# Enigmatisms/AdaPT

Measured on AMD Instinct MI355X. Metric: Msamples/s (W*H*spp/s), unidirectional MIS path tracing, higher is better.
Workload: dtype f32

## Files before the change

### adapt_amd/_lib.py

```python
from __future__ import annotations

import ctypes as C
import os

_HERE = os.path.dirname(os.path.abspath(__file__))
LIB_PATHS = {"fast": os.environ.get("ADAPT_MI_LIB") or os.path.join(_HERE, "libadapt_mi.so"),
             "exact": os.environ.get("ADAPT_MI_LIB_EXACT") or os.path.join(_HERE, "libadapt_mi_exact.so")}
_variant = "exact" if os.environ.get("APT_EXACT", "0") not in ("", "0") else "fast"
LIB_PATH = LIB_PATHS[_variant]

f32p = C.POINTER(C.c_float)
i32p = C.POINTER(C.c_int32)
u32p = C.POINTER(C.c_uint32)
u8p = C.POINTER(C.c_uint8)
f64p = C.POINTER(C.c_double)
APT_N_KERNELS = 5
KERNEL_NAMES = ("generate", "extend", "shade", "shadow", "finalize")


class AptError(RuntimeError):
    pass


class SceneDesc(C.Structure):
# ... 58 lines not shown
    "apt_read_pixels": (C.c_int, [C.c_void_p, f32p]),
    "apt_get_accum": (C.c_int, [C.c_void_p, f32p, i32p]),
    "apt_set_accum": (C.c_int, [C.c_void_p, f32p, C.c_int32]),
    "apt_reset": (C.c_int, [C.c_void_p]),
    "apt_read_transient": (C.c_int, [C.c_void_p, f32p]),
    "apt_set_transient": (C.c_int, [C.c_void_p, f32p]),
    "apt_read_sample_counts": (C.c_int, [C.c_void_p, i32p, u8p]),
    "apt_read_moments": (C.c_int, [C.c_void_p, f64p]),
    "apt_set_adaptive_state": (C.c_int, [C.c_void_p, i32p, f64p, u8p]),
    "apt_get_stats": (C.c_int, [C.c_void_p, C.POINTER(Stats)]),
    "apt_device_ptr": (C.c_int, [C.c_void_p, C.POINTER(C.c_void_p), i32p]),
    "apt_stream": (C.c_int, [C.c_void_p, C.POINTER(C.c_void_p)]),
    "apt_intersect": (C.c_int, [C.c_void_p, C.c_int32, f32p, f32p, i32p, f32p, f32p]),
    "apt_occluded": (C.c_int, [C.c_void_p, C.c_int32, f32p, f32p, f32p, i32p]),
    "apt_rng_stream": (C.c_int, [C.c_int32, C.c_uint32, C.c_uint32, C.c_uint32, C.c_int32, u32p]),
    "apt_bxdf_probe": (C.c_int, [C.c_int32, C.c_int32, i32p, f32p, f32p, C.c_float, C.c_int32, C.c_uint32, f32p]),
    "apt_medium_probe": (C.c_int, [C.c_int32, C.c_int32, i32p, f32p, C.c_int32, f32p, C.c_uint32, f32p]),
    "apt_volume_probe": (C.c_int, [C.c_int32, C.c_int32, i32p, f32p, f32p, C.c_int32, f32p, C.c_uint32, f32p]),
    "apt_emitter_probe": (C.c_int, [C.c_void_p, C.c_int32, f32p, C.c_uint32, f32p]),
    "apt_texture_probe": (C.c_int, [C.c_void_p, C.c_int32, i32p, f32p, f32p]),
    "apt_transient_bin_probe": (C.c_int, [C.c_int32, C.c_int32, f32p, C.c_float, C.c_float, C.c_int32, i32p]),
    "apt_renderer_info": (C.c_int, [C.c_void_p, i32p, i32p, C.POINTER(C.c_int64), i32p, C.POINTER(C.c_char_p), i32p]),
    "apt_renderer_camera_fused": (C.c_int, [C.c_void_p, i32p]),
    "apt_measure_sclk_mhz": (C.c_int, [C.c_int32, f32p]),
    "apt_last_error": (C.c_char_p, []),
    "apt_version": (C.c_char_p, []),
}

_libs = {}


def use(variant: str) -> str:
    global _variant, LIB_PATH
    if variant not in LIB_PATHS:
        raise ValueError(f"unknown build variant {variant!r}")
    prev, _variant = _variant, variant
    LIB_PATH = LIB_PATHS[variant]
    return prev


def variant() -> str:
    return _variant


def load(variant: str | None = None):
    v = variant or _variant
# ... 28 lines not shown
```

### adapt_amd/csrc/api.hip

```cpp
#include <hip/hip_runtime.h>
#include <chrono>

#include <algorithm>
#include <cmath>
#include <cstdio>
#include <cstdlib>
#include <cstring>
#include <limits>
#include <memory>
#include <string>
#include <vector>

#include "../../include/adapt_mi.h"
#include "bvh_build.hpp"
#include "shade_stage.hpp"
#include "unit_kernels.hpp"
#include "volumetric.hpp"

#define APT_EXPORT extern "C" __attribute__((visibility("default")))

static thread_local std::string g_err;
static int fail(int code, const std::string& msg) { g_err = msg; return code; }
#define HIP_TRY(expr)                                                                              \
    do {                                                                                           \
// ... 130 lines not shown
struct EventPair { hipEvent_t a, b; int kernel; bool own_a; };

struct Lane {
    hipStream_t stream = nullptr;
    DevBuf pool, counters, ovf;
    Queues q{};
    hipEvent_t fin = nullptr;
    LdsPlan plan{};
    Counters* cnt() const { return counters.as<Counters>(); }
};

struct apt_renderer {
    const apt_scene* scene = nullptr;
    apt_render_cfg cfg{};
    Params par{};
    int n_cols = 0, npix = 0, spp_batch = 1;
    int cnt = 0;
    std::vector<Lane> lanes;
    int n_lanes = 1;
    hipStream_t stream() const { return lanes[0].stream; }
    DevBuf accum, scratch, pix_key;
    DevBuf cam_strips;
    int camera_fuse = 0;
    Counters host_counters{};
    int grid_small = 0, grid_trace = 0, nq = APT_MAX_NQ;
    const ShadeVariant* shade = nullptr;
    int trace_mode = 0;
    int trace_nt = BLOCK;
    int trace_items = BLOCK;
    int sorted = 0;
    int volumetric = 0;
    int dyn_fetch = 0;
    bool tile_ok = false;
    extend_fn extend = nullptr, fix = nullptr;
    int ovf_levels = 0;
    int v_ncls = 0;
    int vev_single = 0;
    vev_shade_fn vev_all = nullptr;
    bool vev_live[APT_MAX_CLASSES] = {};
    vev_group_fn vgroup_fn[APT_N_VGROUPS] = {};
    int vgroup_cls[APT_N_VGROUPS][4] = {};
    group_fn group_fn_[APT_N_GROUPS] = {};
    int group_cls[APT_N_GROUPS][APT_GROUP_SLOTS] = {};
    std::string shade_name;
    size_t lds_bytes = 0, lds_bytes_any = 0;
    int grid_shadow = 0;
// ... 554 lines not shown
    r->extend = r->dyn_fetch ? kExtendDyn[r->sorted] : (r->trace_mode == 3 ? kExtendFlatHot[r->sorted] : kExtend[r->trace_mode][r->sorted]);
    r->fix = kFixFlat[r->sorted];
    return APT_OK;
}

static apt::CamFilm cam_film(const apt_render_cfg& c) {
    apt::CamFilm cf;
    memcpy(cf.cam_r, c.cam_r, sizeof(cf.cam_r)); memcpy(cf.cam_t, c.cam_t, sizeof(cf.cam_t));
    cf.inv_focal = c.inv_focal; cf.half_w = c.half_w; cf.half_h = c.half_h;
    cf.width = c.width; cf.height = c.height; cf.n_cols = owned_columns(c); cf.band_width = c.band_width; cf.rank = c.rank; cf.world = c.world_size;
    return cf;
}
static int make_camera_strips(apt_renderer* r) {
    if (r->par.fused != 2) return APT_OK;
    const apt_scene* sc = r->scene;
    const bool cull = !(getenv("APT_CAMERA_CULL") && atoi(getenv("APT_CAMERA_CULL")) == 0);
    std::vector<uint64_t> masks;
    if (apt::camera_strips(sc->h_prims.data(), sc->n_prims, sc->h_flat_recs, sc->h_flat_tab, sc->h_flat_counts, cam_film(r->cfg), cull, masks) != 0)
        return fail(APT_E_INVALID, "apt_renderer_create: camera strip lists: bad record or film");
    hipError_t e = upload(r->cam_strips, masks);
    if (e != hipSuccess) return fail(APT_E_HIP, std::string("upload camera strip lists: ") + hipGetErrorString(e));
    const bool want = !(getenv("APT_CAMERA_FUSE") && atoi(getenv("APT_CAMERA_FUSE")) == 0);
    r->camera_fuse = (want && !r->adaptive && !r->par.do_crop && r->par.max_bounce >= 1 && r->shade->traced_cam != nullptr) ? 1 : 0;
    return APT_OK;
}

APT_EXPORT int apt_camera_strips(const float* prims, int32_t n_prims, const int32_t* obj_info, int32_t n_objects, const apt_render_cfg* cfg, int32_t cull,
                                 uint64_t* masks, int32_t masks_cap, int32_t* n_strips, int32_t* n_pairs) {
    if (!prims || !obj_info || !cfg || n_prims <= 0 || n_objects <= 0 || !n_strips || !n_pairs) return fail(APT_E_INVALID, "apt_camera_strips: bad argument");
    apt_render_cfg c = *cfg;
    if (c.world_size <= 0) { c.world_size = 1; c.rank = 0; }
    if (c.band_width <= 0) c.band_width = c.width;
    if (c.width <= 0 || c.height <= 0 || c.rank < 0 || c.rank >= c.world_size || owned_columns(c) <= 0) return fail(APT_E_INVALID, "apt_camera_strips: bad film or rank");
    std::vector<float> st, tb; int cn[7];
    if (apt::build_flat(prims, n_prims, obj_info, n_objects, nullptr, st, tb, cn) != 0) return fail(APT_E_INVALID, "apt_camera_strips: obj_info range outside the primitive array");
    std::vector<uint64_t> m;
    if (apt::camera_strips(prims, n_prims, st, tb, cn, cam_film(c), cull != 0, m) != 0) return fail(APT_E_INVALID, "apt_camera_strips: bad record or film");
    *n_strips = (int32_t)m.size();
    *n_pairs = (cn[0] + cn[1] + 1) / 2 + (cn[2] + cn[3] + 1) / 2 + (cn[4] + cn[5] + 1) / 2 + (cn[6] + 1) / 2;
    if (masks) { if (masks_cap < (int32_t)m.size()) return fail(APT_E_INVALID, "apt_camera_strips: masks buffer too small"); memcpy(masks, m.data(), m.size() * 8); }
    return APT_OK;
}

static int make_lanes(apt_renderer* r) {
    const apt_scene* sc = r->scene;
    const Params& p = r->par;
// ... 203 lines not shown
    if (c.band_width <= 0) c.band_width = c.width;
    if (c.rank < 0 || c.rank >= c.world_size) return fail(APT_E_INVALID, "apt_renderer_create: rank outside world_size");
    if (c.device != sc->device) return fail(APT_E_INVALID, "apt_renderer_create: renderer and scene must live on the same device");
    if (c.transient_bins < 0) return fail(APT_E_INVALID, "apt_renderer_create: transient_bins must be >= 0 (0 = steady state)");
    if (c.transient_bins > 0) {
        if (c.volumetric) return fail(APT_E_INVALID, "apt_renderer_create: transient rendering is a surface-renderer mode (volumetric = 0)");
        if (c.num_shadow_ray > 4) return fail(APT_E_INVALID, "apt_renderer_create: transient rendering takes at most 4 light samples per vertex (num_shadow_ray <= 4)");
        if (c.world_size > 1) return fail(APT_E_INVALID, "apt_renderer_create: transient rendering runs on one rank (world_size = 1)");
        if (!(c.transient_interval > 0.f) || !std::isfinite(c.transient_interval) || !std::isfinite(c.transient_min_time))
            return fail(APT_E_INVALID, "apt_renderer_create: transient_interval must be positive and finite, transient_min_time finite");
    }
    if (!std::isfinite(c.adaptive_threshold)) return fail(APT_E_INVALID, "apt_renderer_create: adaptive_threshold must be finite (> 0: adaptive sampling, <= 0: off)");
    if (c.adaptive_threshold > 0.f) {
        if (c.transient_bins > 0)
            return fail(APT_E_INVALID, "apt_renderer_create: adaptive sampling and transient rendering do not combine (transient_bins must be 0 when adaptive_threshold > 0)");
        if (c.adaptive_min_spp <= 0 || c.adaptive_step <= 0)
            return fail(APT_E_INVALID, "apt_renderer_create: adaptive sampling needs adaptive_min_spp > 0 and adaptive_step > 0");
    }
    HIP_TRY(hipSetDevice(c.device));
    apt_renderer* r = new apt_renderer();
    struct Owner { apt_renderer* r; ~Owner() { if (r) apt_renderer_destroy(r); } } owner{r};
    r->scene = sc; r->cfg = c;
    r->adaptive = c.adaptive_threshold > 0.f ? 1 : 0;
    if (int rc = plan_film(r)) return rc;
    pick_traversal(r);
    if (int rc = pick_shading(r)) return rc;
    if (int rc = make_camera_strips(r)) return rc;
    if (int rc = make_lanes(r)) return rc;
    if (int rc = make_transient(r)) return rc;
    if (int rc = make_adaptive(r)) return rc;
    if (int rc = plan_lds_and_grids(r)) return rc;
    if (int rc = make_overflow_stacks(r)) return rc;
    for (Lane& ln : r->lanes) HIP_TRY(hipStreamSynchronize(ln.stream));
    owner.r = nullptr;
    *out = r;
    return APT_OK;
}

static int grid_for(size_t n, int cap_blocks, int nq, int nt = BLOCK) {
    size_t b = (n + nt - 1) / nt;
    b = ((b + nq - 1) / nq) * nq;
    if (b < (size_t)nq) b = nq;
    return (int)(b < (size_t)cap_blocks ? b : (size_t)cap_blocks);
}

static void unchain(apt_renderer* r, hipStream_t st) {
// ... 32 lines not shown
        r->kernel_ms[ev.kernel] += ms;
    }
    for (auto& ev : r->pending) { if (ev.own_a) r->free_events.push_back(ev.a); r->free_events.push_back(ev.b); }
    r->pending.clear();
    r->chain.clear();
    if (r->render_pending) {
        float ms = 0.f;
        HIP_TRY(hipEventElapsedTime(&ms, r->ev_r0, r->ev_r1));
        r->render_ms += ms; r->render_pending = false;
    }
    return APT_OK;
}

static int lane_batch(const apt_renderer* r, int32_t n_spp) {
    if (n_spp <= 0) return 1;
    int n_batches = (n_spp + r->spp_batch - 1) / r->spp_batch;
    n_batches = ((n_batches + r->n_lanes - 1) / r->n_lanes) * r->n_lanes;
    return std::max(1, std::min(r->spp_batch, (n_spp + n_batches - 1) / n_batches));
}

static int begin_batch(apt_renderer* r, Lane& ln) {
    unchain(r, ln.stream);
    HIP_TRY(hipMemsetAsync(ln.cnt(), 0, offsetof(Counters, stats), ln.stream));
    return APT_OK;
}
static void launch_extend(apt_renderer* r, Lane& ln, const Params& p, size_t total, int cur) {
    const DevScene& sc = r->scene->dev;
    Counters* cnt = ln.cnt();
    { LaunchTimer t(r, 1, ln.stream); hipLaunchKernelGGL(r->extend, dim3(grid_for(total, r->grid_trace, r->nq, r->trace_items)), dim3(r->trace_nt), r->lds_bytes, ln.stream, sc, p, ln.q, cnt, cur, (const uint32_t*)cnt->n_active[cur], ln.plan); }
    if (r->trace_mode == 3) { LaunchTimer t(r, 1, ln.stream, false); hipLaunchKernelGGL(r->fix, dim3(r->grid_fix), dim3(BLOCK), 0, ln.stream, sc, p, ln.q, cnt, cur, (const uint32_t*)cnt->n_active[cur], ln.plan); }
}
static int finalize_batch(apt_renderer* r, Lane& ln, const Params& p, hipEvent_t& prev_fin) {
    if (prev_fin && r->n_lanes > 1) { unchain(r, ln.stream); HIP_TRY(hipStreamWaitEvent(ln.stream, prev_fin, 0)); }
    {
        LaunchTimer t(r, 4, ln.stream);
        if (r->adaptive) hipLaunchKernelGGL(k_finalize_ad, dim3(grid_for((size_t)r->npix, r->grid_small, 1)), dim3(BLOCK), 0, ln.stream, p, ln.q, r->accum.as<float>(), r->aq);
        else hipLaunchKernelGGL(k_finalize, dim3(grid_for((size_t)r->npix, r->grid_small, 1)), dim3(BLOCK), 0, ln.stream, p, ln.q, r->accum.as<float>());
    }
    HIP_TRY(hipEventRecord(ln.fin, ln.stream));
    prev_fin = ln.fin;
    HIP_TRY(hipGetLastError());
    return APT_OK;
}

static int render_volumetric(apt_renderer* r, int32_t n_spp) {
    const DevScene& sc = r->scene->dev;
// ... 539 lines not shown
    int ndev = 0;
    if (int rc = count_device(&ndev)) return rc;
    if (device < 0 || device >= ndev) return fail(APT_E_INVALID, "apt_measure_sclk_mhz: device ordinal out of range");
    HIP_TRY(hipSetDevice(device));
    hipDeviceProp_t prop;
    HIP_TRY(hipGetDeviceProperties(&prop, device));
    const int grid = std::max(1, prop.multiProcessorCount) * 8, n_waves = grid * (BLOCK / 64);
    DevBuf out, sink;
    HIP_TRY(out.alloc((size_t)n_waves * 16)); HIP_TRY(sink.alloc(16));
    for (int pass = 0; pass < 2; pass++) {
        hipLaunchKernelGGL(k_clock_probe, dim3(grid), dim3(BLOCK), 0, 0, 20000, 1.0f, out.as<unsigned long long>(), sink.as<float>());
        HIP_TRY(hipGetLastError());
        HIP_TRY(hipDeviceSynchronize());
    }
    std::vector<unsigned long long> h((size_t)n_waves * 2);
    HIP_TRY(hipMemcpy(h.data(), out.p, h.size() * 8, hipMemcpyDeviceToHost));
    std::vector<double> r;
    for (int w = 0; w < n_waves; w++) if (h[2 * (size_t)w + 1] > 0) r.push_back(100.0 * (double)h[2 * (size_t)w] / (double)h[2 * (size_t)w + 1]);
    if (r.empty()) return fail(APT_E_STATE, "apt_measure_sclk_mhz: the wall clock did not advance");
    std::nth_element(r.begin(), r.begin() + r.size() / 2, r.end());
    *mhz = (float)r[r.size() / 2];
    return APT_OK;
}
APT_EXPORT int apt_renderer_camera_fused(const apt_renderer* r, int32_t* fused) {
    if (!r || !fused) return fail(APT_E_INVALID, "apt_renderer_camera_fused: null argument");
    *fused = r->camera_fuse;
    return APT_OK;
}
APT_EXPORT int apt_renderer_info(const apt_renderer* r, int32_t* spp_batch, int32_t* n_subqueues, int64_t* queue_bytes, int32_t* lds_bytes, const char** shade_variant, int32_t* trace_mode) {
    if (!r) return fail(APT_E_INVALID, "apt_renderer_info: null handle");
    if (spp_batch) *spp_batch = r->spp_batch;
    if (n_subqueues) *n_subqueues = r->nq;
    if (queue_bytes) *queue_bytes = (int64_t)r->lanes[0].pool.bytes * (int64_t)r->lanes.size();
    if (lds_bytes) *lds_bytes = (int32_t)r->lds_bytes;
    if (shade_variant) *shade_variant = r->shade_name.c_str();
    if (trace_mode) *trace_mode = r->trace_mode;
    return APT_OK;
}
```

### adapt_amd/csrc/shade_stage.hpp

```cpp
#pragma once
#include "stages.hpp"

APT_D float ti_fmod(float a, float b) { float q = floorf(a / b); return a - b * q; }
APT_D f3 mix3(f3 a, f3 b, float t) { return a * (1.0f - t) + b * t; }
APT_D f3 texture_query(const DevScene& sc, int map, int obj, float u, float v) {
    const int* ti_ = sc.tex_i + 15 * obj + 5 * map; const float* tf = sc.tex_f + 6 * obj + 2 * map;
    const float w = (float)ti_[3], h = (float)ti_[4];
    const float scaled_u = ti_fmod((u * tf[0]) * w, w - 1.f), scaled_v = ti_fmod((v * tf[1]) * h, h - 1.f);
    float floor_u = floorf(scaled_u), floor_v = floorf(scaled_v);
    const float ratio_u = scaled_u - floor_u, ratio_v = scaled_v - floor_v;
    floor_u = floor_u + (float)ti_[1]; floor_v = floor_v + (float)ti_[2];
    const int fu = (int)floor_u, fv = (int)floor_v;
    const float* img = sc.atlas[map]; const int W = sc.atlas_w[map];
    const float* r0 = img + ((size_t)fv * W + fu) * 3; const float* r1 = r0 + (size_t)W * 3;
    const f3 q_ff = mk3(r0[0], r0[1], r0[2]), q_cf = mk3(r0[3], r0[4], r0[5]), q_fc = mk3(r1[0], r1[1], r1[2]), q_cc = mk3(r1[3], r1[4], r1[5]);
    return mix3(mix3(q_ff, q_cf, ratio_u), mix3(q_fc, q_cc, ratio_u), ratio_v);
}
APT_D bool get_uv_item(const DevScene& sc, int map, int obj, int prim, float bu, float bv, f3& out) {
    if (sc.atlas[map] == nullptr || !(sc.tex_i[15 * obj + 5 * map] > -255)) return false;
    const float* uv = sc.uvs + 6 * prim;
    const float w0 = 1.f - bu - bv;
    const float gu = (uv[2] * bu + uv[4] * bv) + uv[0] * w0, gv = (uv[3] * bu + uv[5] * bv) + uv[1] * w0;
    out = texture_query(sc, map, obj, gu, gv);
    return true;
// ... 37 lines not shown
        if (lane_id() == 0) old = atomicMax(&cnt->fix_claim[sq * CNT_PAD], epoch);
        old = (uint32_t)__builtin_amdgcn_readlane((int)old, 0);
    }
    if (old >= epoch) {
        while (__hip_atomic_load(&cnt->fix_done[sq * CNT_PAD], __ATOMIC_ACQUIRE, __HIP_MEMORY_SCOPE_AGENT) < epoch) __builtin_amdgcn_s_sleep(16);
        return;
    }
    const uint32_t qbase = (uint32_t)sq * p.subcap, sh_qbase = (uint32_t)sq * q.sh_subcap;
    const bool need_uv = sc.has_vn || sc.tex_i != nullptr;
    for (uint32_t base = 0; base < n_def; base += 64u) {
        const uint32_t li = base + lane_id(); const bool valid = li < n_def;
        const uint32_t lj = valid ? li : n_def - 1u;
        const uint32_t io = (q.tr_stage_top ? qbase + p.subcap - n_def + lj : (uint32_t)ncls * p.cap + qbase + lj) << 4;
        const float4 ra = ldq(q.tr[cur][0], io), rb = ldq(q.tr[cur][1], io), rc = ldq(q.tr[cur][2], io), rd = ldq(q.tr[cur][3], io);
        const f3 o = mk3(ra.x, ra.y, ra.z), d = mk3(rb.x, rb.y, rb.z);
        HitRec r0, r1; r0.t = r1.t = 1e7f; r0.prim = r1.prim = -1; r0.u = r0.v = r1.u = r1.v = 0.f;
        int c0, c1;
        flat_closest2(sc.flat, sc.sweep, sc.prim_class, o, d, o, d, r0, r1, c0, c1);
        if (valid && r0.prim >= 0) {
            const int oc = ncls > 1 ? c0 : 0;
            const uint32_t pos = atomicAdd(&cnt->n_tr[bounce % 3][oc][sq * CNT_PAD], 1u);
            const uint32_t slot = (uint32_t)oc * p.cap + qbase + pos, so = slot << 4;
            stq(q.tr[cur][0], so, make_float4(ra.x, ra.y, ra.z, r0.t));
            stq(q.tr[cur][1], so, make_float4(rb.x, rb.y, rb.z, __uint_as_float((__float_as_uint(rb.w) & ~0xffu) | (uint32_t)r0.prim)));
            stq(q.tr[cur][2], so, rc); stq(q.tr[cur][3], so, rd);
            if (need_uv) { float2 uv_; uv_.x = r0.u; uv_.y = r0.v; stq(q.tr_uv[cur], slot << 3, uv_); }
        } else if (valid && !(rd.x == 0.f && rd.y == 0.f && rd.z == 0.f)) {
            const uint32_t id = __float_as_uint(rc.w), lp_ = id & ((1u << p.pix_bits) - 1u), s_ = id >> p.pix_bits;
            add_radiance(q.L, p.cap, (s_ * (uint32_t)p.npix + lp_) << 2, mk3(rd.x, rd.y, rd.z), true);
        }
    }
    uint32_t t_lit = 0;
    for (uint32_t base = 0; base < n_sh; base += 64u) {
        const uint32_t li = base + lane_id(); const bool valid = li < n_sh;
        const uint32_t io = (sh_qbase + (valid ? li : n_sh - 1u)) << 2;
        const f3 o = ld3q(q.sh_o, q.sh_cap, io), d = ld3q(q.sh_d, q.sh_cap, io), c = ld3q(q.sh_c, q.sh_cap, io);
        const float dist = ldq(q.sh_tmax, io); const uint32_t slot = ldq(q.sh_id, io);
        bool occ, occ_b;
        const float lim = (dist > 0.0f) ? dist - 1e-4f : 1e7f;
        flat_any2(sc.flat, sc.sweep, o, d, o, d, lim, lim, occ, occ_b);
        const bool weird = !(isfinite(c.x) && isfinite(c.y) && isfinite(c.z));
        const bool add = valid && (!occ || weird);
        for (unsigned long long m = __ballot(add); m != 0ull; m &= m - 1ull) {
            if ((int)lane_id() == __ffsll((long long)m) - 1) add_radiance(q.L, p.cap, slot, occ ? c * 0.f : c, true);
        }
        t_lit += (valid && !occ) ? 1u : 0u;
    }
    flush_stat(t_lit, &cnt->stats[sq][ST_LIT]);
    if (lane_id() == 0) __hip_atomic_store(n_sh_p, 0u, __ATOMIC_RELAXED, __HIP_MEMORY_SCOPE_AGENT);
    __threadfence();
    if (lane_id() == 0) __hip_atomic_store(&cnt->fix_done[sq * CNT_PAD], epoch, __ATOMIC_RELEASE, __HIP_MEMORY_SCOPE_AGENT);
}
// ... 153 lines not shown
    uint32_t n, cam_total = 0;
    if constexpr (CAM) {
        cam_total = (uint32_t)(A_->p).npix * (uint32_t)(A_->p).spp_batch;
        const uint32_t n_waves = (cam_total + 63u) / 64u, nq_ = (uint32_t)(A_->p).nq;
        n = n_waves > (uint32_t)sl.q ? ((n_waves - (uint32_t)sl.q + nq_ - 1u) / nq_) * 64u : 0u;
    } else {
        fix_prologue((A_->sc), (A_->p), (A_->q), cnt, cur, sl.q, bounce);
        n = __hip_atomic_load(&cnt->n_tr[bounce % 3][0][sl.q * CNT_PAD], __ATOMIC_RELAXED, __HIP_MEMORY_SCOPE_AGENT);
    }
    uint32_t pf_pm = 0;
    auto prefetch_prim = [&](uint32_t b) { pf_pm = ldq(reinterpret_cast<const uint32_t*>(trB), ((qbase + min(b + threadIdx.x, n - 1u)) << 4) + 12u); };
    if (PFP && n > 0) prefetch_prim(sl.first);
    for (uint32_t base = sl.first; base < n; base += sl.stride) {
        APT_ARGS_PHASE();
        const uint32_t pos = base + threadIdx.x, idx = qbase + pos;
        bool alive = pos < n;
        const uint32_t cu_pm = pf_pm;
        float4 cu_ra = make_float4(0.f, 0.f, 0.f, 0.f), cu_rb = cu_ra;
        if (PFP) { const int rp = max(tr_prim(cu_pm), 0); cu_ra = (A_->sc).prim_shade[2 * rp]; cu_rb = (A_->sc).prim_shade[2 * rp + 1]; prefetch_prim(base + sl.stride); }
        Vertex vx; vertex_reset(vx);
        Rng rng; rng_init(rng, 0u, 0u, 0u, 0u);
        f3 Lc = splat3(0.f);
        bool entry = alive;
        float ray_pdf = 1.f;
        if constexpr (CAM) {
            const uint32_t w = (uint32_t)__builtin_amdgcn_readfirstlane((int)(pos >> 6)) * (uint32_t)(A_->p).nq + (uint32_t)sl.q;
            const uint32_t id_ = w * 64u + lane_id();
            const bool valid = alive && id_ < cam_total;
            f3 dir = mk3(0.f, 0.f, 1.f);
            uint32_t draws = 0;
            uint32_t jitter_tail[2] = {0u, 0u};
            if (valid) {
                const uint32_t lp = id_ % (uint32_t)(A_->p).npix, s = id_ / (uint32_t)(A_->p).npix;
                int i, j; local_to_global((A_->p), lp, i, j);
                for (int pl = 0; pl < (A_->p).l_planes; pl++) stL((A_->q).L, (A_->p).cap, (id_ << 2) | (uint32_t)pl, splat3(0.f));
                dir = camera_ray_dir((A_->p), i, j, s, draws, (WINDOW && APT_DRAW_WINDOW_CARRY) ? jitter_tail : nullptr);
                vx.id = (s << (A_->p).pix_bits) | lp;
            }
            if (draws) atomicAdd(&s_draws[threadIdx.x >> 6], draws);
            const f3 cam_o = mk3((A_->p).cam_t[0], (A_->p).cam_t[1], (A_->p).cam_t[2]);
            float c_t = 0.f; int c_run = -1, c_idx = -1;
            if (__any(valid)) c_idx = flat_closest1<true>((A_->sc).flat, cam_o, dir, 1e7f, c_t, c_run, camera_strip_mask((A_->p), strips, w));
            const bool c_defer = valid && (c_run >= 0 || flat_needs_cull((A_->sc).flat, dir));
            HitRec hr; hr.t = 1e7f; hr.prim = -1; hr.u = hr.v = 0.f;
            int hit_cls = 0;
            if (valid && !c_defer && c_idx >= 0) flat_resolve((A_->sc).flat, c_idx, c_t, cam_o, dir, hr, hit_cls);
            { const uint32_t nv = wave_count(valid); t_samples += nv; t_extend += nv; }
            if (__any(c_defer)) {
                const int ncls = (A_->q).tr_ncls;
                const uint32_t dpos = wave_append(c_defer, &cnt->n_tr[0][ncls][sl.q * CNT_PAD]);
                if (c_defer) {
                    const uint32_t slot = (A_->q).tr_stage_top ? qbase + (A_->p).subcap - 1u - dpos : (uint32_t)ncls * (A_->p).cap + qbase + dpos, so = slot << 4;
                    stq((A_->q).tr[0][0], so, make_float4(cam_o.x, cam_o.y, cam_o.z, hr.t));
                    stq((A_->q).tr[0][1], so, make_float4(dir.x, dir.y, dir.z, __uint_as_float(tr_pack(hr.prim, draws, false))));
                    stq((A_->q).tr[0][2], so, make_float4(1.f, 1.f, 1.f, __uint_as_float(vx.id)));
                    float one = 1.f;
                    if (WINDOW) asm volatile("" : "+v"(one));
                    stq((A_->q).tr[0][3], so, make_float4(0.f, 0.f, 0.f, one));
                    if ((A_->sc).has_vn || (A_->sc).tex_i != nullptr) { float2 uv_; uv_.x = hr.u; uv_.y = hr.v; stq((A_->q).tr_uv[0], slot << 3, uv_); }
                }
            }
            entry = valid && !c_defer;
            alive = entry && hr.prim >= 0;
            if (alive) {
                vx.o = cam_o; vx.d = dir; vx.thr = splat3(1.f);
                f3 rec_kd; float2 uv; uv.x = hr.u; uv.y = hr.v;
                build_hit((A_->sc), hr.prim, hr.t, uv.x, uv.y, vx.o, vx.d, vx.it, vx.hit_light, rec_kd);
                alive = open_vertex<BM, SM, TEX>(A_, vx, rng, hr.prim, rec_kd, tr_meta(tr_pack(hr.prim, draws, false), 0u), ray_pdf, uv, 0, (WINDOW && APT_DRAW_WINDOW_CARRY) ? jitter_tail : nullptr);
            }
        }
        if (!CAM && alive && bounce > 0) { const float4 dd = ldq(trD, idx << 4); Lc = mk3(dd.x, dd.y, dd.z); if (SM & 2) ray_pdf = dd.w; }
        if (!CAM && alive) {
            const float4 a = ldq(trA, idx << 4), b_ = ldq(trB, idx << 4), c = ldq(trC, idx << 4);
            vx.o = mk3(a.x, a.y, a.z); vx.d = mk3(b_.x, b_.y, b_.z); vx.thr = mk3(c.x, c.y, c.z); vx.id = __float_as_uint(c.w);
            const uint32_t pm = PFP ? cu_pm : __float_as_uint(b_.w);
            const int prim = tr_prim(pm);
            if (prim < 0) alive = false;
            else {
                f3 rec_kd; float2 uv; uv.x = uv.y = 0.f;
                if ((A_->sc).has_vn || (TEX && (A_->sc).tex_i != nullptr)) uv = ldq((A_->q).tr_uv[cur], idx << 3);
                if (PFP) build_hit_rec((A_->sc), cu_ra, cu_rb, prim, a.w, uv.x, uv.y, vx.o, vx.d, vx.it, vx.hit_light, rec_kd);
                else build_hit((A_->sc), prim, a.w, uv.x, uv.y, vx.o, vx.d, vx.it, vx.hit_light, rec_kd);
                alive = open_vertex<BM, SM, TEX>(A_, vx, rng, prim, rec_kd, tr_meta(pm, (uint32_t)bounce), ray_pdf, uv, bounce);
            }
        }
        tl.shade += wave_count(alive);
#ifdef APT_NEAR_STATS
        t_near += wave_count(alive && bounce > 0 && vx.it.min_depth < 2e-3f);
#endif
        if (alive) vx.hit_point = vx.d * vx.it.min_depth + vx.o;

        APT_ARGS_PHASE();
        bool break_flag = false;
        DevSrc src_only;
        if ((A_->sc).n_sources == 1) src_only = ld_src_uniform((A_->sc).src);
        const LightSample f = sample_light<BM, SM, false>(A_, vx, rng, geom, src_only, alive, break_flag);
        if (f.poisoned) Lc = splat3(f.mis_w);
        tl.shadow += wave_count(f.sampled); tl.poison += wave_count(f.poisoned);
        int occ_e = 0;
        if ((A_->sc).n_sources != 1) {
            const unsigned long long wm = __ballot(f.want);
            occ_e = -1;
            if (wm != 0ull) {
                const int e0 = __builtin_amdgcn_readlane(f.src, __ffsll((long long)wm) - 1);
                if (!__any(f.want && f.src != e0)) occ_e = e0;
            }
        }
        APT_ARGS_PHASE();
        bool cont = false, is_spec = false;
        f3 new_d = mk3(0.f, 1.f, 0.f);
        float new_pdf = 1.f;
        if (alive) {
            new_d = emit_and_scatter<BM, SM>(A_, vx, rng, new_pdf, is_spec, [&](f3 add) { Lc = Lc + add; });
            cont = (bounce + 1) < (A_->p).max_bounce;
        }
        if (rng.draw != vx.draw0) atomicAdd(&s_draws[threadIdx.x >> 6], rng.draw - vx.draw0);
        APT_ARGS_PHASE();
        float tr_t = 0.f; int tr_hit = -1; float tr_u = 0.f, tr_v = 0.f; int tr_q = -1;
        TrAppend tr_app; tr_app.raw = 0u; tr_app.rank = 0u;
        {
            int tr_idx = -1, tr_run = -1, hit_cls = 0;
            if (__any(cont)) tr_idx = flat_closest1((A_->sc).flat, vx.hit_point, new_d, 1e7f, tr_t, tr_run);
            const bool tr_defer = cont && (tr_run >= 0 || flat_needs_cull((A_->sc).flat, new_d));
            t_extend += wave_count(cont);
            cont = cont && (tr_idx >= 0 || tr_defer);
            if (cont && !tr_defer) { HitRec hr; flat_resolve((A_->sc).flat, tr_idx, tr_t, vx.hit_point, new_d, hr, hit_cls); tr_hit = hr.prim; tr_u = hr.u; tr_v = hr.v; }
            tr_q = !cont ? -1 : (tr_defer ? 1 : 0);
            { const Append a_ = append_issue(tr_q == 0, next_counter); tr_app.raw = a_.raw; tr_app.rank = rank_in(a_.m); }
        }
        APT_ARGS_PHASE();
        {
            const bool defer = f.want && flat_needs_cull((A_->sc).flat, f.dir);
            bool occ = false;
            if (__any(f.want && !defer)) {
                const FlatList ls = (occ_e >= 0) ? flat_occ_list((A_->sc).flat, occ_e) : flat_full_list((A_->sc).flat);
                occ = flat_any1(ls, vx.hit_point, f.dir, (f.dist > 0.0f) ? f.dist - 1e-4f : 1e7f);
            }
            if (__any(defer)) {
                const uint32_t spos = wave_append(defer, &cnt->n_fix_sh[cur][sl.q * CNT_PAD]);
                if (defer && spos < (A_->q).sh_subcap) { const uint32_t so = (sh_qbase + spos) << 2; shadow_store((A_->q), so, vx.hit_point, f.dir, f.dist, f.contrib); stq((A_->q).sh_id, so, vx.l_off); }
            }
            const bool traced = f.want && !defer;
            if (traced) {
                const bool weird = !(isfinite(f.contrib.x) && isfinite(f.contrib.y) && isfinite(f.contrib.z));
                if (!occ || weird) Lc = Lc + (occ ? f.contrib * 0.f : f.contrib);
            }
            t_traced += wave_count(f.want); t_lit += wave_count(traced && !occ);
        }
        uint32_t npos = (uint32_t)__builtin_amdgcn_readlane((int)tr_app.raw, 0) + tr_app.rank;
        if (__any(tr_q == 1)) { const uint32_t dpos = wave_append(tr_q == 1, next_counter + APT_MAX_NQ * CNT_PAD); if (tr_q == 1) npos = dpos; }
        if (cont) {
            const uint32_t slot = (tr_q == 1) ? qbase + (A_->p).subcap - 1u - npos : qbase + npos, so = slot << 4;
            stq((A_->q).tr[nxt][0], so, make_float4(vx.hit_point.x, vx.hit_point.y, vx.hit_point.z, tr_t));
            stq((A_->q).tr[nxt][1], so, make_float4(new_d.x, new_d.y, new_d.z, __uint_as_float(tr_pack(tr_hit, rng.draw, is_spec))));
            stq((A_->q).tr[nxt][2], so, make_float4(vx.thr.x, vx.thr.y, vx.thr.z, __uint_as_float(vx.id)));
            stq((A_->q).tr[nxt][3], so, make_float4(Lc.x, Lc.y, Lc.z, new_pdf));
            if ((A_->sc).has_vn || (A_->sc).tex_i != nullptr) { float2 uv_; uv_.x = tr_u; uv_.y = tr_v; stq((A_->q).tr_uv[nxt], slot << 3, uv_); }
        }
        if (!cont && entry && !(Lc.x == 0.f && Lc.y == 0.f && Lc.z == 0.f)) {
            const uint32_t lp_ = vx.id & ((1u << (A_->p).pix_bits) - 1u), s_ = vx.id >> (A_->p).pix_bits;
            add_radiance((A_->q).L, (A_->p).cap, (s_ * (uint32_t)(A_->p).npix + lp_) << 2, Lc, true);
        }
    }
    flush_uniform(t_traced, &cnt->stats[sl.q][ST_SHADOW_TRACED]); flush_uniform(t_lit, &cnt->stats[sl.q][ST_LIT]);
    flush_uniform(t_extend, &cnt->stats[sl.q][ST_EXTEND]);
    if (CAM) flush_uniform(t_samples, &cnt->stats[sl.q][ST_SAMPLES]);
    tally_flush(tl, s_draws, cnt, sl.q);
#ifdef APT_NEAR_STATS
    flush_uniform(t_near, &cnt->stats[sl.q][14]);
#endif
}
#endif
template <int BM, int SM, int TEX, bool CQ, bool TR = false>
APT_D void shade_staged(args3_ptr A0, Counters* cnt, const ShadeIn& in, int cur, int bounce, TransQ tq = TransQ{}) {
    const ShadeArgs3* A_ = args_fresh(A0);
    const int nxt = cur ^ 1;
    const SubLoop sl = sub_loop((A_->p).nq);
    const uint32_t n = in.counts[sl.q * CNT_PAD];
    const uint32_t qbase = (uint32_t)sl.q * (A_->p).subcap, sh_qbase = (uint32_t)sl.q * (A_->q).sh_subcap;
    uint32_t* next_counter = &cnt->n_active[nxt][sl.q * CNT_PAD];
    uint32_t* shadow_counter = &cnt->n_shadow[sl.q * CNT_PAD];
    const EmitterGeom geom = {(A_->sc).precom, (A_->sc).normals, (A_->sc).obj_info};
    __shared__ uint32_t s_draws[BLOCK / 64];
    if (lane_id() == 0) s_draws[threadIdx.x >> 6] = 0;
// ... 164 lines not shown
```

### adapt_amd/csrc/stages.hpp

```cpp
#pragma once
#include <hip/hip_runtime.h>

#include "rng.hpp"
#include "shading.hpp"
#include "traverse.hpp"
#include "vec.hpp"

struct DevMedium {
    int type;
    float ior;
    f3 u_s, u_a, u_e, par, pdf;
};
struct DevVolume {
    int type, xres, yres, zres;
    f3 albedo, trans, mini, maxi, majorant, pdf;
    f3 inv_r0, inv_r1, inv_r2;
    DevMedium ph;
    const float* grid;
};
struct DevScene {
    DevBvh bvh;
    SweepScene sweep;
    FlatScene flat;
    const float* normals;
// ... 21 lines not shown
    float cam_r[9], cam_t[3];
    float inv_focal, half_w, half_h;
    int W, H, n_cols, npix;
    int band_width, rank, world;
    int do_crop, sx, ex, sy, ey;
    int max_bounce, S;
    float inv_S;
    int use_rr, use_mis, anti_alias, stratified, two_sides, rr_bounce_th;
    float rr_threshold;
    uint32_t seed;
    int cnt_base, spp_batch;
    uint32_t cap;
    uint32_t subcap;
    int nq;
    uint32_t pix_bits;
    const uint32_t* pix_key;
    float inv_ns, inv_ns1;
    int fix_par;
    int volumetric_flat;
    int nee_vm;
    int l_planes;
    int fused;
    float w_min[3], w_max[3];
};

struct Queues {
    float* ray_o[2]; float* ray_d[2];
    float* hit_t; int* hit_prim; float* hit_u; float* hit_v;
    float4* tr[2][4]; float2* tr_uv[2]; int tr_ncls, tr_stage_top;
    uint32_t* fix_ext; uint32_t* fix_sh;
    float* thr[2]; uint32_t* id[2]; uint32_t* meta[2]; float* pdf[2];
    float* sh_o; float* sh_d; float* sh_tmax; float* sh_c; uint32_t* sh_id;
    uint32_t* sh_walk[2];
    float* L;
    uint32_t sh_cap, sh_subcap;
    float4* cq[4];
    int n_classes;
};
#define APT_MAX_CLASSES 8
struct TransQ {
    float* t_path;
    float4* emit;
    float* t_light;
    float4* bins;
    int n_bins;
    float min_time, interval, max_time;
};
// ... 10 lines not shown

#ifndef APT_MAX_NQ
#define APT_MAX_NQ 32
#endif
#define CNT_PAD 32
enum { ST_SAMPLES = 0, ST_EXTEND, ST_SHADE, ST_SHADOW, ST_SHADOW_TRACED, ST_LIT, ST_DRAWS, ST_POISON, ST_TRACK, ST_OVERFLOW, ST_COUNT };
struct Counters {
    uint32_t n_active[2][APT_MAX_NQ * CNT_PAD];
    uint32_t n_shadow[APT_MAX_NQ * CNT_PAD];
    uint32_t n_walk[8][APT_MAX_NQ * CNT_PAD];
    uint32_t n_cls[8][APT_MAX_NQ * CNT_PAD];
    uint32_t n_fix_ext[2][APT_MAX_NQ * CNT_PAD];
    uint32_t n_fix_sh[2][APT_MAX_NQ * CNT_PAD];
    uint32_t n_work[2][APT_MAX_NQ * CNT_PAD];
    uint32_t n_tr[3][8 + 1][APT_MAX_NQ * CNT_PAD];
    uint32_t fix_claim[APT_MAX_NQ * CNT_PAD];
    uint32_t fix_done[APT_MAX_NQ * CNT_PAD];
    unsigned long long stats[APT_MAX_NQ][16];
#ifdef APT_WALK_STATS
    unsigned long long wdbg[2][8];
#endif
};

APT_D uint32_t pack_meta(uint32_t draw, uint32_t bounce, bool spec) { return (draw & 0xffffu) | ((bounce & 0xffu) << 16) | (spec ? (1u << 24) : 0u); }

#define BLOCK 256
#define TR_NO_PRIM 0xffu
APT_D uint32_t tr_pack(int prim, uint32_t draw, bool spec) { return (prim < 0 ? TR_NO_PRIM : (uint32_t)prim) | ((draw & 0xffffu) << 8) | (spec ? (1u << 24) : 0u); }
APT_D int tr_prim(uint32_t pm) { return ((pm & 0xffu) == TR_NO_PRIM) ? -1 : (int)(pm & 0xffu); }
APT_D uint32_t tr_meta(uint32_t pm, uint32_t bounce) { return pack_meta(pm >> 8, bounce, ((pm >> 24) & 1u) != 0u); }
#ifndef APT_EXCLUSIVE_L
#define APT_EXCLUSIVE_L(p) ((p).S == 1 || (p).l_planes == (p).S)
#endif

struct LdsPlan { int stack_depth; uint2* ovf; int ovf_stride; };
extern __shared__ float4 s_dyn[];
typedef __attribute__((address_space(3))) float lds_f;
APT_D TravStack make_stack(const LdsPlan& plan) {
    TravStack ts;
    ts.lds = (lds_u2*)(reinterpret_cast<grp_t*>(s_dyn)) + threadIdx.x;
    ts.stride = BLOCK; ts.k = plan.stack_depth; ts.ovf_stride = plan.ovf_stride;
    ts.ovf = plan.ovf ? (glb_u2*)(reinterpret_cast<grp_t*>(plan.ovf) + (blockIdx.x * blockDim.x + threadIdx.x)) : (glb_u2*)nullptr;
    ts.lut = (lds_u8*)nullptr;
    return ts;
}
APT_D TravStack make_walk_stack(const LdsPlan& plan) {
    TravStack ts = make_stack(plan);
    ts.lut = (lds_u8*)(reinterpret_cast<float*>(s_dyn) + (size_t)plan.stack_depth * BLOCK * 2 + 6 * BLOCK);
    fill_permute_lut(ts.lut);
    __syncthreads();
    return ts;
}

// ... 840 lines not shown
```

### adapt_amd/renderer.py

```python
from __future__ import annotations

import ctypes as C
import time
from typing import List, Optional

import numpy as np

from . import _lib
from .scene_pack import FlatScene, RenderConfig, make_config, pack_scene
from .tiles import TilePlan

__all__ = ["Renderer", "VolumeRenderer", "DeviceScene", "bxdf_probe", "medium_probe", "volume_probe", "rng_stream", "adaptive_config", "adaptive_segments", "relative_error"]

ADAPTIVE_DEFAULTS = {"min_spp": 64, "step": 32}


def adaptive_config(adaptive) -> Optional[dict]:
    if adaptive is None or adaptive is False:
        return None
    if not isinstance(adaptive, dict):
        raise TypeError("adaptive must be None or a dict {'threshold': t, 'min_spp': 64, 'step': 32}")
    unknown = set(adaptive) - {"threshold", "min_spp", "step"}
    if unknown:
        raise ValueError(f"adaptive: unknown key(s) {sorted(unknown)}")
# ... 377 lines not shown
        return occ

    def emitter_probe(self, in11, seed: int = 0) -> np.ndarray:
        x = np.ascontiguousarray(in11, np.float32).reshape(-1, 11)
        out = np.zeros((x.shape[0], 12), np.float32)
        _lib.check(self.lib.apt_emitter_probe(self.scene.handle, x.shape[0], _fp(x), int(seed) & 0xffffffff, _fp(out)), "apt_emitter_probe", self.lib)
        return out

    def info(self) -> dict:
        b, nq, lds, tm = C.c_int32(0), C.c_int32(0), C.c_int32(0), C.c_int32(0)
        qb = C.c_int64(0)
        name = C.c_char_p()
        _lib.check(self.lib.apt_renderer_info(self.handle, C.byref(b), C.byref(nq), C.byref(qb), C.byref(lds), C.byref(name), C.byref(tm)), "apt_renderer_info", self.lib)
        return {"spp_per_batch": b.value, "n_subqueues": nq.value, "queue_bytes": qb.value, "lds_bytes": lds.value,
                "shade_variant": name.value.decode() if name.value else "",
                "traversal": {0: "bvh", 1: "sweep", 2: "tile", 3: "flat"}.get(tm.value, str(tm.value)), "arithmetic": self.arithmetic,
                "sampling": "adaptive" if self.adaptive else "uniform", **({"adaptive": dict(self.adaptive)} if self.adaptive else {})}

    def camera_fused(self) -> bool:
        f = C.c_int32(0)
        _lib.check(self.lib.apt_renderer_camera_fused(self.handle, C.byref(f)), "apt_renderer_camera_fused", self.lib)
        return bool(f.value)

    def get_check_point(self) -> dict:
        return {"w": self.w, "h": self.h, "crop_x": self.crop_x, "crop_y": self.crop_y, "crop_rx": self.crop_rx,
                "crop_ry": self.crop_ry, "focal": self.focal, "num_objects": self.num_objects, "num_prims": self.num_prims,
                "cam_orient": np.array(self.cam_orient), "src_num": self.src_num, "cam_t": np.array(self.cam_t),
                "accumulation": self.color.to_numpy(), "counter": self._cnt,
                **({"transient_bins": self.tile_transient()} if self.n_bins else {}),
                **(self._adaptive_check_point() if self.adaptive else {})}

    _ADAPTIVE_KEYS = ("adaptive", "sample_counts", "moments", "active")

    def _adaptive_check_point(self) -> dict:
        n, act = self.tile_sample_counts(with_mask=True)
        return {"adaptive": dict(self.adaptive), "sample_counts": n, "moments": self.tile_moments(), "active": act}

    def load_check_point(self, check_point: dict):
        if self.adaptive and "moments" not in check_point:
            raise ValueError("this checkpoint has no per-pixel moments (a uniform render's): an adaptive renderer cannot continue it")
        if not self.adaptive and any(k in check_point for k in self._ADAPTIVE_KEYS):
            raise ValueError("this checkpoint is an adaptive render's: continue it with Renderer(..., adaptive=...)")
        for key, val in check_point.items():
            if key in ("accumulation", "counter", "transient_bins") + self._ADAPTIVE_KEYS:
                continue
            if key in ("cam_t", "cam_orient"):
# ... 38 lines not shown
```

### include/adapt_mi.h

```cpp
#ifndef ADAPT_MI_H
#define ADAPT_MI_H

#include <stdint.h>

#ifdef __cplusplus
extern "C" {
#endif

#define APT_OK            0
#define APT_E_INVALID    -1
#define APT_E_NO_DEVICE  -2
#define APT_E_HIP        -3
#define APT_E_NOMEM      -4
#define APT_E_STATE      -5

typedef struct apt_bvh apt_bvh;
typedef struct apt_scene apt_scene;
typedef struct apt_renderer apt_renderer;

typedef struct apt_scene_desc {
    int32_t n_prims, n_objects, n_sources, has_vertex_normal;
    const float*   prims;
    const float*   normals;
    const float*   v_normals;
// ... 98 lines not shown
int apt_read_sample_counts(apt_renderer*, int32_t* counts, uint8_t* active);
int apt_read_moments(apt_renderer*, double* s2);
int apt_set_adaptive_state(apt_renderer*, const int32_t* counts, const double* s2, const uint8_t* active);
int apt_get_stats(apt_renderer*, apt_stats* out);
int apt_device_ptr(apt_renderer*, void** accum_dev, int32_t* cnt);
int apt_stream(apt_renderer*, void** hip_stream);

int apt_intersect(apt_renderer*, int32_t n, const float* o, const float* d,
                  int32_t* prim_out, float* t_out, float* uv_out);
int apt_occluded(apt_renderer*, int32_t n, const float* o, const float* d, const float* tmax, int32_t* occ_out);
int apt_rng_stream(int32_t device, uint32_t pixel, uint32_t seed, uint32_t sample, int32_t n, uint32_t* out);
int apt_bxdf_probe(int32_t device, int32_t n, const int32_t* bxdf_i, const float* bxdf_f, const float* dirs12,
                   float world_ior, int32_t do_sample, uint32_t seed, float* out);
int apt_texture_probe(const apt_scene*, int32_t n, const int32_t* map_obj, const float* uv, float* out3);
int apt_medium_probe(int32_t device, int32_t n, const int32_t* med_i, const float* med_f, int32_t mode, const float* in7,
                     uint32_t seed, float* out8);
int apt_volume_probe(int32_t device, int32_t n, const int32_t* vol_i, const float* vol_f, const float* vol_grid, int32_t mode,
                     const float* in10, uint32_t seed, float* out8);
int apt_emitter_probe(const apt_scene*, int32_t n, const float* in11, uint32_t seed, float* out12);
int apt_transient_bin_probe(int32_t device, int32_t n, const float* t, float min_time, float interval, int32_t n_bins, int32_t* out);
int apt_renderer_info(const apt_renderer*, int32_t* spp_batch, int32_t* n_subqueues, int64_t* queue_bytes,
                      int32_t* lds_bytes, const char** shade_variant, int32_t* trace_mode);
int apt_renderer_camera_fused(const apt_renderer*, int32_t* fused);

int apt_measure_sclk_mhz(int32_t device, float* mhz);

const char* apt_last_error(void);
const char* apt_version(void);

#ifdef __cplusplus
}
#endif
#endif
```

Before: 6160.

## Track radiance-slot liveness to skip camera zeroing and read-modify-write of L

Adds a live bit to the packed prim/meta word that marks whether a path's radiance slot has been written. With l_store enabled (the default when camera fusion is on), the camera stage no longer zeroes every L plane. The first writer stores radiance directly instead of loading and accumulating, and a zero is written only when a deferred shadow contribution will later be added. This cuts global memory traffic on the L buffer at the cost of extra branching and an added invariant on the bit encoding. A poison-fill debug option and probe APIs are added for validation.

```diff
diff --git a/adapt_amd/_lib.py b/adapt_amd/_lib.py
--- a/adapt_amd/_lib.py
+++ b/adapt_amd/_lib.py
@@ -104,6 +104,8 @@
     "apt_transient_bin_probe": (C.c_int, [C.c_int32, C.c_int32, f32p, C.c_float, C.c_float, C.c_int32, i32p]),
     "apt_renderer_info": (C.c_int, [C.c_void_p, i32p, i32p, C.POINTER(C.c_int64), i32p, C.POINTER(C.c_char_p), i32p]),
     "apt_renderer_camera_fused": (C.c_int, [C.c_void_p, i32p]),
+    "apt_renderer_radiance_stored": (C.c_int, [C.c_void_p, i32p]),
+    "apt_tr_pm_probe": (C.c_int, [C.c_int32, C.c_uint32, C.c_int32, C.c_int32, C.c_int32, C.c_uint32, u32p]),
     "apt_measure_sclk_mhz": (C.c_int, [C.c_int32, f32p]),
     "apt_last_error": (C.c_char_p, []),
     "apt_version": (C.c_char_p, []),
diff --git a/adapt_amd/csrc/api.hip b/adapt_amd/csrc/api.hip
--- a/adapt_amd/csrc/api.hip
+++ b/adapt_amd/csrc/api.hip
@@ -176,6 +176,7 @@
     DevBuf accum, scratch, pix_key;
     DevBuf cam_strips;
     int camera_fuse = 0;
+    int l_poison = 0;
     Counters host_counters{};
     int grid_small = 0, grid_trace = 0, nq = APT_MAX_NQ;
     const ShadeVariant* shade = nullptr;
@@ -776,6 +777,8 @@
     if (e != hipSuccess) return fail(APT_E_HIP, std::string("upload camera strip lists: ") + hipGetErrorString(e));
     const bool want = !(getenv("APT_CAMERA_FUSE") && atoi(getenv("APT_CAMERA_FUSE")) == 0);
     r->camera_fuse = (want && !r->adaptive && !r->par.do_crop && r->par.max_bounce >= 1 && r->shade->traced_cam != nullptr) ? 1 : 0;
+    const bool want_store = !(getenv("APT_L_STORE") && atoi(getenv("APT_L_STORE")) == 0);
+    r->par.l_store = (want_store && r->camera_fuse) ? 1 : 0;
     return APT_OK;
 }
 
@@ -1025,6 +1028,7 @@
     struct Owner { apt_renderer* r; ~Owner() { if (r) apt_renderer_destroy(r); } } owner{r};
     r->scene = sc; r->cfg = c;
     r->adaptive = c.adaptive_threshold > 0.f ? 1 : 0;
+    r->l_poison = (getenv("APT_L_POISON") && atoi(getenv("APT_L_POISON")) != 0) ? 1 : 0;
     if (int rc = plan_film(r)) return rc;
     pick_traversal(r);
     if (int rc = pick_shading(r)) return rc;
@@ -1103,6 +1107,7 @@
 static int begin_batch(apt_renderer* r, Lane& ln) {
     unchain(r, ln.stream);
     HIP_TRY(hipMemsetAsync(ln.cnt(), 0, offsetof(Counters, stats), ln.stream));
+    if (r->l_poison) { unchain(r, ln.stream); HIP_TRY(hipMemsetAsync(ln.q.L, 0x71, (size_t)16 * r->par.cap * (size_t)r->par.l_planes, ln.stream)); }
     return APT_OK;
 }
 static void launch_extend(apt_renderer* r, Lane& ln, const Params& p, size_t total, int cur) {
@@ -1688,6 +1693,18 @@
     *mhz = (float)r[r.size() / 2];
     return APT_OK;
 }
+APT_EXPORT int apt_renderer_radiance_stored(const apt_renderer* r, int32_t* stored) {
+    if (!r || !stored) return fail(APT_E_INVALID, "apt_renderer_radiance_stored: null argument");
+    *stored = r->par.l_store;
+    return APT_OK;
+}
+APT_EXPORT int apt_tr_pm_probe(int32_t prim, uint32_t draw, int32_t spec, int32_t live, int32_t new_prim, uint32_t bounce, uint32_t* out) {
+    if (!out || prim < -1 || prim >= (int32_t)TR_NO_PRIM || new_prim < 0 || new_prim >= (int32_t)TR_NO_PRIM) return fail(APT_E_INVALID, "apt_tr_pm_probe: bad argument");
+    const uint32_t pm = tr_mark_live(tr_pack(prim, draw, spec != 0), live != 0), pm2 = tr_with_prim(pm, new_prim);
+    out[0] = pm; out[1] = (uint32_t)tr_prim(pm); out[2] = tr_meta(pm, bounce); out[3] = tr_live(pm) ? 1u : 0u;
+    out[4] = pm2; out[5] = (uint32_t)tr_prim(pm2); out[6] = tr_meta(pm2, bounce); out[7] = tr_live(pm2) ? 1u : 0u;
+    return APT_OK;
+}
 APT_EXPORT int apt_renderer_camera_fused(const apt_renderer* r, int32_t* fused) {
     if (!r || !fused) return fail(APT_E_INVALID, "apt_renderer_camera_fused: null argument");
     *fused = r->camera_fuse;
diff --git a/adapt_amd/csrc/shade_stage.hpp b/adapt_amd/csrc/shade_stage.hpp
--- a/adapt_amd/csrc/shade_stage.hpp
+++ b/adapt_amd/csrc/shade_stage.hpp
@@ -83,12 +83,14 @@
             const uint32_t pos = atomicAdd(&cnt->n_tr[bounce % 3][oc][sq * CNT_PAD], 1u);
             const uint32_t slot = (uint32_t)oc * p.cap + qbase + pos, so = slot << 4;
             stq(q.tr[cur][0], so, make_float4(ra.x, ra.y, ra.z, r0.t));
-            stq(q.tr[cur][1], so, make_float4(rb.x, rb.y, rb.z, __uint_as_float((__float_as_uint(rb.w) & ~0xffu) | (uint32_t)r0.prim)));
+            stq(q.tr[cur][1], so, make_float4(rb.x, rb.y, rb.z, __uint_as_float(tr_with_prim(__float_as_uint(rb.w), r0.prim))));
             stq(q.tr[cur][2], so, rc); stq(q.tr[cur][3], so, rd);
             if (need_uv) { float2 uv_; uv_.x = r0.u; uv_.y = r0.v; stq(q.tr_uv[cur], slot << 3, uv_); }
-        } else if (valid && !(rd.x == 0.f && rd.y == 0.f && rd.z == 0.f)) {
-            const uint32_t id = __float_as_uint(rc.w), lp_ = id & ((1u << p.pix_bits) - 1u), s_ = id >> p.pix_bits;
-            add_radiance(q.L, p.cap, (s_ * (uint32_t)p.npix + lp_) << 2, mk3(rd.x, rd.y, rd.z), true);
+        } else if (valid) {
+            const uint32_t id = __float_as_uint(rc.w), lp_ = id & ((1u << p.pix_bits) - 1u), s_ = id >> p.pix_bits, code = (s_ * (uint32_t)p.npix + lp_) << 2;
+            const f3 Lc = mk3(rd.x, rd.y, rd.z);
+            if (p.l_store && !tr_live(__float_as_uint(rb.w))) stL(q.L, p.cap, code, Lc);
+            else if (!(rd.x == 0.f && rd.y == 0.f && rd.z == 0.f)) add_radiance(q.L, p.cap, code, Lc, true);
         }
     }
     uint32_t t_lit = 0;
@@ -288,6 +290,7 @@
         Rng rng; rng_init(rng, 0u, 0u, 0u, 0u);
         f3 Lc = splat3(0.f);
         bool entry = alive;
+        bool live = false;
         float ray_pdf = 1.f;
         if constexpr (CAM) {
             const uint32_t w = (uint32_t)__builtin_amdgcn_readfirstlane((int)(pos >> 6)) * (uint32_t)(A_->p).nq + (uint32_t)sl.q;
@@ -299,7 +302,7 @@
             if (valid) {
                 const uint32_t lp = id_ % (uint32_t)(A_->p).npix, s = id_ / (uint32_t)(A_->p).npix;
                 int i, j; local_to_global((A_->p), lp, i, j);
-                for (int pl = 0; pl < (A_->p).l_planes; pl++) stL((A_->q).L, (A_->p).cap, (id_ << 2) | (uint32_t)pl, splat3(0.f));
+                if (!(A_->p).l_store) for (int pl = 0; pl < (A_->p).l_planes; pl++) stL((A_->q).L, (A_->p).cap, (id_ << 2) | (uint32_t)pl, splat3(0.f));
                 dir = camera_ray_dir((A_->p), i, j, s, draws, (WINDOW && APT_DRAW_WINDOW_CARRY) ? jitter_tail : nullptr);
                 vx.id = (s << (A_->p).pix_bits) | lp;
             }
@@ -341,6 +344,7 @@
             vx.o = mk3(a.x, a.y, a.z); vx.d = mk3(b_.x, b_.y, b_.z); vx.thr = mk3(c.x, c.y, c.z); vx.id = __float_as_uint(c.w);
             const uint32_t pm = PFP ? cu_pm : __float_as_uint(b_.w);
             const int prim = tr_prim(pm);
+            live = tr_live(pm);
             if (prim < 0) alive = false;
             else {
                 f3 rec_kd; float2 uv; uv.x = uv.y = 0.f;
@@ -384,6 +388,7 @@
         APT_ARGS_PHASE();
         float tr_t = 0.f; int tr_hit = -1; float tr_u = 0.f, tr_v = 0.f; int tr_q = -1;
         TrAppend tr_app; tr_app.raw = 0u; tr_app.rank = 0u;
+        bool fresh = false;
         {
             int tr_idx = -1, tr_run = -1, hit_cls = 0;
             if (__any(cont)) tr_idx = flat_closest1((A_->sc).flat, vx.hit_point, new_d, 1e7f, tr_t, tr_run);
@@ -406,6 +411,7 @@
                 const uint32_t spos = wave_append(defer, &cnt->n_fix_sh[cur][sl.q * CNT_PAD]);
                 if (defer && spos < (A_->q).sh_subcap) { const uint32_t so = (sh_qbase + spos) << 2; shadow_store((A_->q), so, vx.hit_point, f.dir, f.dist, f.contrib); stq((A_->q).sh_id, so, vx.l_off); }
             }
+            fresh = (A_->p).l_store != 0 && defer && !live;
             const bool traced = f.want && !defer;
             if (traced) {
                 const bool weird = !(isfinite(f.contrib.x) && isfinite(f.contrib.y) && isfinite(f.contrib.z));
@@ -418,14 +424,24 @@
         if (cont) {
             const uint32_t slot = (tr_q == 1) ? qbase + (A_->p).subcap - 1u - npos : qbase + npos, so = slot << 4;
             stq((A_->q).tr[nxt][0], so, make_float4(vx.hit_point.x, vx.hit_point.y, vx.hit_point.z, tr_t));
-            stq((A_->q).tr[nxt][1], so, make_float4(new_d.x, new_d.y, new_d.z, __uint_as_float(tr_pack(tr_hit, rng.draw, is_spec))));
+            stq((A_->q).tr[nxt][1], so, make_float4(new_d.x, new_d.y, new_d.z, __uint_as_float(tr_mark_live(tr_pack(tr_hit, rng.draw, is_spec), live || fresh))));
             stq((A_->q).tr[nxt][2], so, make_float4(vx.thr.x, vx.thr.y, vx.thr.z, __uint_as_float(vx.id)));
             stq((A_->q).tr[nxt][3], so, make_float4(Lc.x, Lc.y, Lc.z, new_pdf));
             if ((A_->sc).has_vn || (A_->sc).tex_i != nullptr) { float2 uv_; uv_.x = tr_u; uv_.y = tr_v; stq((A_->q).tr_uv[nxt], slot << 3, uv_); }
         }
-        if (!cont && entry && !(Lc.x == 0.f && Lc.y == 0.f && Lc.z == 0.f)) {
-            const uint32_t lp_ = vx.id & ((1u << (A_->p).pix_bits) - 1u), s_ = vx.id >> (A_->p).pix_bits;
-            add_radiance((A_->q).L, (A_->p).cap, (s_ * (uint32_t)(A_->p).npix + lp_) << 2, Lc, true);
+        {
+            bool put = !cont && entry;
+            f3 out = Lc;
+            const uint32_t lp_ = vx.id & ((1u << (A_->p).pix_bits) - 1u), s_ = vx.id >> (A_->p).pix_bits, code = (s_ * (uint32_t)(A_->p).npix + lp_) << 2;
+            if (put && (live || !(A_->p).l_store)) {
+                put = !(Lc.x == 0.f && Lc.y == 0.f && Lc.z == 0.f);
+                if (put) { const f3 a = ldL((A_->q).L, (A_->p).cap, code); out = mk3(a.x + Lc.x, a.y + Lc.y, a.z + Lc.z); }
+            } else if (!put && fresh) {
+                float zero = 0.f;
+                asm volatile("" : "+v"(zero));
+                out = splat3(zero); put = true;
+            }
+            if (put) stL((A_->q).L, (A_->p).cap, code, out);
         }
     }
     flush_uniform(t_traced, &cnt->stats[sl.q][ST_SHADOW_TRACED]); flush_uniform(t_lit, &cnt->stats[sl.q][ST_LIT]);
diff --git a/adapt_amd/csrc/stages.hpp b/adapt_amd/csrc/stages.hpp
--- a/adapt_amd/csrc/stages.hpp
+++ b/adapt_amd/csrc/stages.hpp
@@ -67,7 +67,9 @@
     int l_planes;
     int fused;
     float w_min[3], w_max[3];
+    int l_store;
 };
+static_assert(sizeof(Params) == 240, "Params::l_store is meant to fill the tail padding: the kernel-argument layout of every kernel stays as it was");
 
 struct Queues {
     float* ray_o[2]; float* ray_d[2];
@@ -124,13 +126,17 @@
 #endif
 };
 
-APT_D uint32_t pack_meta(uint32_t draw, uint32_t bounce, bool spec) { return (draw & 0xffffu) | ((bounce & 0xffu) << 16) | (spec ? (1u << 24) : 0u); }
+APT_HD uint32_t pack_meta(uint32_t draw, uint32_t bounce, bool spec) { return (draw & 0xffffu) | ((bounce & 0xffu) << 16) | (spec ? (1u << 24) : 0u); }
 
 #define BLOCK 256
 #define TR_NO_PRIM 0xffu
-APT_D uint32_t tr_pack(int prim, uint32_t draw, bool spec) { return (prim < 0 ? TR_NO_PRIM : (uint32_t)prim) | ((draw & 0xffffu) << 8) | (spec ? (1u << 24) : 0u); }
-APT_D int tr_prim(uint32_t pm) { return ((pm & 0xffu) == TR_NO_PRIM) ? -1 : (int)(pm & 0xffu); }
-APT_D uint32_t tr_meta(uint32_t pm, uint32_t bounce) { return pack_meta(pm >> 8, bounce, ((pm >> 24) & 1u) != 0u); }
+APT_HD uint32_t tr_pack(int prim, uint32_t draw, bool spec) { return (prim < 0 ? TR_NO_PRIM : (uint32_t)prim) | ((draw & 0xffffu) << 8) | (spec ? (1u << 24) : 0u); }
+APT_HD int tr_prim(uint32_t pm) { return ((pm & 0xffu) == TR_NO_PRIM) ? -1 : (int)(pm & 0xffu); }
+APT_HD uint32_t tr_meta(uint32_t pm, uint32_t bounce) { return pack_meta(pm >> 8, bounce, ((pm >> 24) & 1u) != 0u); }
+#define TR_LIVE (1u << 25)
+APT_HD bool tr_live(uint32_t pm) { return (pm & TR_LIVE) != 0u; }
+APT_HD uint32_t tr_mark_live(uint32_t pm, bool live) { return pm | (live ? TR_LIVE : 0u); }
+APT_HD uint32_t tr_with_prim(uint32_t pm, int prim) { return (pm & ~0xffu) | (uint32_t)prim; }
 #ifndef APT_EXCLUSIVE_L
 #define APT_EXCLUSIVE_L(p) ((p).S == 1 || (p).l_planes == (p).S)
 #endif
diff --git a/adapt_amd/renderer.py b/adapt_amd/renderer.py
--- a/adapt_amd/renderer.py
+++ b/adapt_amd/renderer.py
@@ -423,6 +423,11 @@
         _lib.check(self.lib.apt_renderer_camera_fused(self.handle, C.byref(f)), "apt_renderer_camera_fused", self.lib)
         return bool(f.value)
 
+    def radiance_stored(self) -> bool:
+        f = C.c_int32(0)
+        _lib.check(self.lib.apt_renderer_radiance_stored(self.handle, C.byref(f)), "apt_renderer_radiance_stored", self.lib)
+        return bool(f.value)
+
     def get_check_point(self) -> dict:
         return {"w": self.w, "h": self.h, "crop_x": self.crop_x, "crop_y": self.crop_y, "crop_rx": self.crop_rx,
                 "crop_ry": self.crop_ry, "focal": self.focal, "num_objects": self.num_objects, "num_prims": self.num_prims,
diff --git a/include/adapt_mi.h b/include/adapt_mi.h
--- a/include/adapt_mi.h
+++ b/include/adapt_mi.h
@@ -144,6 +144,8 @@
 int apt_renderer_info(const apt_renderer*, int32_t* spp_batch, int32_t* n_subqueues, int64_t* queue_bytes,
                       int32_t* lds_bytes, const char** shade_variant, int32_t* trace_mode);
 int apt_renderer_camera_fused(const apt_renderer*, int32_t* fused);
+int apt_renderer_radiance_stored(const apt_renderer*, int32_t* stored);
+int apt_tr_pm_probe(int32_t prim, uint32_t draw, int32_t spec, int32_t live, int32_t new_prim, uint32_t bounce, uint32_t* out);
 
 int apt_measure_sclk_mhz(int32_t device, float* mhz);
 
```

After: 6225 (median of 2 runs). Within noise of the previous version (+1.1%).
